# pythonmailer/financial-rag-system

Hardware: AMD Instinct MI355X
Metric: queries/sec + recall@5, batch=32 over 10Mx384 corpus (higher is better)
Workload: dtype fp16

## Files before the change

### financial-rag-system_amd/csrc/certify_kernels.hip

```cpp
namespace ragmi {

constexpr int kCandCap = 256;
constexpr int kBandLists = 32;
constexpr int kBandLists6 = 128;

template <typename IdT>
__device__ __forceinline__ void merge4_top32(const float (&ws)[4][32], const IdT (&wi)[4][32],
                                             int lane, IdT none, float& s, IdT& id) {
  s = lane < 32 ? ws[0][lane] : kNegInf;
  id = lane < 32 ? wi[0][lane] : none;
  for (int v = 1; v < 4; ++v) {
    if (lane >= 32) {
      s = ws[v][63 - lane];
      id = wi[v][63 - lane];
    }
    bitonic_merge64(s, id, lane);
  }
}

template <int D, int NC>
__device__ __forceinline__ void exact_scores_pairs(const half8* __restrict__ corpus,
                                                   const int (&rows)[NC],
                                                   const int (&qoff)[NC],
                                                   const float* __restrict__ qn, int lane,
                                                   float (&out)[NC],
                                                   const float* __restrict__ rows32) {
  constexpr int S = steps<D>();
  double acc[NC];
#pragma unroll
  for (int i = 0; i < NC; ++i) acc[i] = 0.0;
  for (int c = lane; c < D / 8; c += 64) {
    float h[NC][8];
#pragma unroll
    for (int i = 0; i < NC; ++i) {
      const int row = rows[i] < 0 ? 0 : rows[i];
      if (rows32) {
        const float4* p = reinterpret_cast<const float4*>(rows32 + (int64_t)row * D + 8 * c);
        const float4 u = p[0], v = p[1];
        h[i][0] = u.x; h[i][1] = u.y; h[i][2] = u.z; h[i][3] = u.w;
        h[i][4] = v.x; h[i][5] = v.y; h[i][6] = v.z; h[i][7] = v.w;
      } else {
        const half8 x =
            corpus[(int64_t)(row >> 4) * (S * 64) + (c >> 2) * 64 + (c & 3) * 16 + (row & 15)];
#pragma unroll
        for (int j = 0; j < 8; ++j) h[i][j] = (float)x[j];
      }
    }
#pragma unroll
    for (int i = 0; i < NC; ++i) {
      const float* qq = qn + qoff[i];
      const float4 qa = *reinterpret_cast<const float4*>(qq + 8 * c);
      const float4 qb = *reinterpret_cast<const float4*>(qq + 8 * c + 4);
      double x = acc[i];
      x = fma((double)h[i][0], (double)qa.x, x);
      x = fma((double)h[i][1], (double)qa.y, x);
      x = fma((double)h[i][2], (double)qa.z, x);
      x = fma((double)h[i][3], (double)qa.w, x);
      x = fma((double)h[i][4], (double)qb.x, x);
      x = fma((double)h[i][5], (double)qb.y, x);
      x = fma((double)h[i][6], (double)qb.z, x);
      x = fma((double)h[i][7], (double)qb.w, x);
      acc[i] = x;
    }
  }
#pragma unroll
  for (int d = 32; d > 0; d >>= 1) {
#pragma unroll
    for (int i = 0; i < NC; ++i) acc[i] = acc[i] + __shfl_xor(acc[i], d, 64);
  }
#pragma unroll
  for (int i = 0; i < NC; ++i)
    out[i] = rows[i] < 0 ? kNegInf : (float)__shfl(acc[i], 0, 64);
}

template <int D, int NC>
__device__ __forceinline__ void exact_scores_wave(const half8* __restrict__ corpus,
                                                  const int (&rows)[NC],
                                                  const float* __restrict__ qq, int lane,
                                                  float (&out)[NC],
                                                  const float* __restrict__ rows32) {
  int qoff[NC];
#pragma unroll
  for (int i = 0; i < NC; ++i) qoff[i] = 0;
  exact_scores_pairs<D, NC>(corpus, rows, qoff, qq, lane, out, rows32);
}

struct ExactStats {
  int* tier;
  unsigned long long* cnt;
  float* t2;
};

template <int D, bool FILTER, int BL = kBandLists>
__global__ __launch_bounds__(256) void select_kernel(const float* __restrict__ part_s,
                                                     const int* __restrict__ part_i,
                                                     const float* __restrict__ heads_s,
                                                     const int* __restrict__ heads_i,
                                                     const int* __restrict__ heads_n,
                                                     int n_lists,
                                                     const half8* __restrict__ corpus,
                                                     const uint32_t* __restrict__ tags,
                                                     const uint32_t* __restrict__ filt,
                                                     const half8* __restrict__ qfrag,
                                                     int n_rows,
                                                     const float* __restrict__ qn, int k,
                                                     const float* __restrict__ eps,
                                                     const float* __restrict__ seed_thr,
                                                     ExactStats fb, int64_t id_offset,
                                                     float* __restrict__ out_s,
                                                     int64_t* __restrict__ out_i,
                                                     int32_t* __restrict__ out_packed,
                                                     const float* __restrict__ rows32,
                                                     const float* __restrict__ eps_t2 = nullptr) {
  __shared__ float w_s[4][32];
  __shared__ int64_t w_i[4][32];
  __shared__ int sel[32];
  __shared__ int sel_n[32];
  __shared__ float cand_s[kCandCap];
  __shared__ int64_t cand_i[kCandCap];
  __shared__ int n_cand;
  __shared__ float head_t;
  __shared__ float c_s[4][32];
  __shared__ int c_i[4][32];
  __shared__ float e_s[32];
  __shared__ int e_i[32];
  __shared__ int qlist[kMaxLists];
  __shared__ int n_q;
  __shared__ int band[BL * kKS];
  __shared__ int n_band;
  __shared__ float n_s[2][32];
  __shared__ int n_i[2][32];
  __shared__ int verdict;
  __shared__ float floor_L, floor_E;
  const int bq = blockIdx.x, grp = bq / kQ, b = bq % kQ;
  const int tid = threadIdx.x, lane = tid & 63, wid = tid >> 6;
  const float eps_q = eps[bq], seed_q = seed_thr[bq];
  part_s += (int64_t)grp * n_lists * (kQ * kKS);
  part_i += (int64_t)grp * n_lists * (kQ * kKS);
  heads_s += (int64_t)grp * kQ * n_lists;
  heads_i += (int64_t)grp * kQ * n_lists;
  heads_n += (int64_t)grp * kQ * n_lists;
  auto at = [&](int l, int pos) { return ((int64_t)l * kQ + b) * kKS + pos; };

  constexpr int kCols = kMaxLists / 256;
  static_assert(kMaxLists <= 2048, "list index packs into 11 bits");
  auto hid = [](int row, int l) { return ((int64_t)row << 11) | (int64_t)l; };
  constexpr int64_t kId64None = INT64_MAX;
  float hs[kCols];
  int64_t hr[kCols];
#pragma unroll
  for (int j = 0; j < kCols; ++j) {
    const int l = min((j * 4 + wid) * 64 + lane, n_lists - 1);
    hs[j] = heads_s[(int64_t)b * n_lists + l];
    hr[j] = hid(heads_i[(int64_t)b * n_lists + l], l);
  }
  float lmax = kNegInf;
#pragma unroll
  for (int j = 0; j < kCols; ++j) {
    const int l = (j * 4 + wid) * 64 + lane;
    const bool ok = l < n_lists && hs[j] != kNegInf;
    hs[j] = ok ? hs[j] : kNegInf;
    hr[j] = ok ? hr[j] : kId64None;
    lmax = fmaxf(lmax, hs[j]);
  }
  {
    float m = lmax;
    int id = tid;
    bitonic_sort64(m, id, lane);
    if (lane < 32) w_s[wid][lane] = m;
  }
  if (tid == 0) {
    n_cand = 0;
    n_q = 0;
    n_band = 0;
    verdict = 0;
  }
  __syncthreads();
  if (wid == 0) {
    float m = lane < 32 ? w_s[0][lane] : kNegInf;
    int id = lane;
    for (int v = 1; v < 4; ++v) {
      if (lane >= 32) {
        m = w_s[v][63 - lane];
        id = 64 * v + lane;
      }
      bitonic_merge64(m, id, lane);
    }
    const float t32 = __shfl(m, 31, 64);
    if (lane == 0) head_t = t32;
  }
  __syncthreads();
  {
    const float T = head_t;
#pragma unroll
    for (int j = 0; j < kCols; ++j) {
      if (hs[j] != kNegInf && hs[j] >= T) {
        const int p = atomicAdd(&n_cand, 1);
        if (p < kCandCap) {
          cand_s[p] = hs[j];
          cand_i[p] = hr[j];
        }
      }
    }
  }
  __syncthreads();
  const int nc = n_cand;
  if (nc <= kCandCap) {
    float m = kNegInf;
    int64_t id = kId64None;
    if (64 * wid + lane < nc) {
      m = cand_s[64 * wid + lane];
// ... 31 lines not shown
      w_i[wid][lane] = ci;
    }
  }
  __syncthreads();
  if (wid == 0) {
    float x;
    int64_t id;
    merge4_top32(w_s, w_i, lane, kId64None, x, id);
    if (lane < 32) {
      const int l = (x != kNegInf) ? (int)(id & 2047) : -1;
      sel[lane] = l;
      sel_n[lane] = l >= 0 ? heads_n[(int64_t)b * n_lists + l] : 0;
    }
  }
  __syncthreads();

  {
    float ls[8];
    int li[8];
#pragma unroll
    for (int j = 0; j < 8; ++j) {
      const int l = sel[wid * 8 + j];
      const int pos = (j == 0 ? lane : 63 - lane) & (kKS - 1);
      const int64_t off = at(l < 0 ? 0 : l, pos);
      ls[j] = part_s[off];
      li[j] = part_i[off];
    }
#pragma unroll
    for (int j = 0; j < 8; ++j) {
      const int pos = (j == 0 ? lane : 63 - lane) & (kKS - 1);
      const bool use = sel[wid * 8 + j] >= 0 && ((j == 0) ? lane < 32 : lane >= 32) &&
                       pos < sel_n[wid * 8 + j];
      ls[j] = use ? ls[j] : kNegInf;
      li[j] = use ? li[j] : kIdNone32;
    }
    float s = ls[0];
    int id = li[0];
#pragma unroll
    for (int j = 1; j < 8; ++j) {
      if (lane >= 32) {
        s = ls[j];
        id = li[j];
      }
      bitonic_merge64(s, id, lane);
    }
    if (lane < 32) {
      c_s[wid][lane] = s;
      c_i[wid][lane] = id;
    }
  }
  __syncthreads();
  if (wid == 0) {
    float s;
    int id;
    merge4_top32(c_s, c_i, lane, kIdNone32, s, id);
    if (lane < 32) {
      c_s[0][lane] = s;
      c_i[0][lane] = id;
    }
  }
  __syncthreads();

  const float* qq = qn + (int64_t)bq * D;
  {
    int rows[8];
    float es[8];
#pragma unroll
    for (int j = 0; j < 8; ++j) {
      const int c = wid * 8 + j;
      rows[j] = c_s[0][c] != kNegInf ? c_i[0][c] : -1;
    }
    exact_scores_wave<D, 8>(corpus, rows, qq, lane, es, rows32);
    if (lane == 0) {
#pragma unroll
      for (int j = 0; j < 8; ++j) {
        e_s[wid * 8 + j] = es[j];
        e_i[wid * 8 + j] = rows[j] >= 0 ? rows[j] : kIdNone32;
      }
    }
  }
  __syncthreads();

  auto emit = [&](float s, int id) {
    if (lane < k) {
      const bool ok = s != kNegInf;
      if (out_packed) {
        out_packed[((int64_t)bq * k + lane) * 2] = __float_as_int(s);
        out_packed[((int64_t)bq * k + lane) * 2 + 1] = ok ? (int32_t)(id + id_offset) : -1;
      } else {
        out_s[(int64_t)bq * k + lane] = s;
        out_i[(int64_t)bq * k + lane] = ok ? (int64_t)id + id_offset : (int64_t)-1;
      }
    }
  };

  float rs = kNegInf;
  int ri = kIdNone32;
  if (wid == 0) {
    if (lane < 32) {
      rs = e_s[lane];
      ri = e_i[lane];
    }
    bitonic_sort64(rs, ri, lane);
    int v = 0;
    {
      const float ek = __shfl(rs, k - 1, 64);
      const float a32 = c_s[0][kKS - 1];
      float L = 0.0f;
      if (!(a32 == kNegInf || ek > a32 + eps_q)) {
        L = ek - eps_q;
        v = (L >= seed_q) ? 1 : 2;
      }
      if (lane == 0) {
        verdict = v;
        floor_L = L;
        floor_E = ek;
      }
    }
    if (v == 0) {
      emit(rs, ri);
      if (lane == 0) fb.tier[bq] = 0;
    }
  }
  __syncthreads();
  if (verdict == 0) return;

  const float L = floor_L;
  const bool seeded = verdict == 1;
  if (seeded) {
#pragma unroll
    for (int j = 0; j < kCols; ++j)
      if (hs[j] != kNegInf && hs[j] >= L) qlist[atomicAdd(&n_q, 1)] = (j * 4 + wid) * 64 + lane;
  }
  __syncthreads();
  const int nql = seeded ? n_q : 0;
  const int a_row = e_i[lane & 31];
  int rnd = 0;
  for (int c0 = 0; c0 < nql; c0 += BL) {
    constexpr int kG = BL / 8;
    const int pos = lane & (kKS - 1);
    float gs[kG];
    int gi[kG], gn[kG];
#pragma unroll
    for (int j = 0; j < kG; ++j) {
      const int l = qlist[min(c0 + (2 * j + (lane >> 5)) * 4 + wid, nql - 1)];
      gs[j] = part_s[at(l, pos)];
      gi[j] = part_i[at(l, pos)];
      gn[j] = heads_n[(int64_t)b * n_lists + l];
    }
#pragma unroll
    for (int j = 0; j < kG; ++j) {
      const bool in = c0 + (2 * j + (lane >> 5)) * 4 + wid < nql && pos < gn[j] && gs[j] >= L;
      if (in && gn[j] >= kKS && pos == kKS - 1) verdict = 2;
      bool in_a = false;
#pragma unroll
      for (int t = 0; t < 32; ++t) in_a |= gi[j] == __builtin_amdgcn_readlane(a_row, t);
      if (in && !in_a) band[atomicAdd(&n_band, 1)] = gi[j];
    }
    __syncthreads();
    if (verdict == 2) break;
    const int nb = n_band;
    for (int r0 = 0; r0 < nb; r0 += 32, ++rnd) {
      int rows[8];
      float es[8];
#pragma unroll
      for (int j = 0; j < 8; ++j) {
        const int c = r0 + wid * 8 + j;
        const int r = band[min(c, nb - 1)];
        rows[j] = c < nb ? r : -1;
      }
      exact_scores_wave<D, 8>(corpus, rows, qq, lane, es, rows32);
      if (lane == 0) {
#pragma unroll
        for (int j = 0; j < 8; ++j) {
          n_s[rnd & 1][wid * 8 + j] = es[j];
          n_i[rnd & 1][wid * 8 + j] = rows[j] >= 0 ? rows[j] : kIdNone32;
        }
      }
      __syncthreads();
      if (wid == 0) {
        if (lane >= 32) {
          rs = n_s[rnd & 1][lane - 32];
          ri = n_i[rnd & 1][lane - 32];
        }
        bitonic_sort64(rs, ri, lane);
      }
    }
    if (c0 + BL < nql) {
      __syncthreads();
      if (tid == 0) n_band = 0;
      __syncthreads();
    }
  }
  if (verdict == 2) {
    if (tid == 0) {
      fb.tier[bq] = 2;
      fb.t2[2 * bq] = eps_t2 ? floor_E - eps_t2[bq] : L;
      fb.t2[2 * bq + 1] = floor_E;
      atomicAdd(&fb.cnt[1], 1ull);
    }
    return;
  }
  if (tid == 0) {
    fb.tier[bq] = 1;
    atomicAdd(&fb.cnt[0], 1ull);
  }
  if (wid == 0) emit(rs, ri);
}

constexpr int kRescanMaxWG = 512;
constexpr int kRescanQ = 16;

__device__ __forceinline__ float exact_tree(double (&p)[16]) {
#pragma unroll
  for (int d = 8; d > 0; d >>= 1) {
#pragma unroll
    for (int i = 0; i < d; ++i) p[i] = p[i] + p[i + d];
  }
  double y = p[0] + __shfl_xor(p[0], 32, 64);
  y = y + __shfl_xor(y, 16, 64);
  return (float)y;
}

template <int D, bool F32>
__device__ __forceinline__ float exact_tile_scores(const half8* __restrict__ corpus,
                                                   const float* __restrict__ rows32, int t,
                                                   const float* __restrict__ qq, int lane) {
  constexpr int S = steps<D>();
  const int h = lane >> 4, r = lane & 15;
  double p[16];
#pragma unroll
  for (int i = 0; i < 16; ++i) p[i] = 0.0;
  int zoff = 0;
  asm volatile("" : "+v"(zoff));
  const half8* tp = corpus + (int64_t)t * (S * 64) + lane;
  const float* rp = F32 ? rows32 + ((int64_t)t * kTileRows + r) * D + 8 * h : nullptr;
  const float* qp = qq + 8 * h;
  constexpr int G = 2;
#pragma unroll
  for (int s0 = 0; s0 < S; s0 += G) {
    float x[G][8];
    float4 qa[G], qb[G];
#pragma unroll
    for (int g = 0; g < G; ++g) {
      const int s = s0 + g;
      if constexpr (F32) {
        const float4 u = *reinterpret_cast<const float4*>(rp + 32 * s + zoff);
        const float4 v = *reinterpret_cast<const float4*>(rp + 32 * s + 4 + zoff);
        x[g][0] = u.x; x[g][1] = u.y; x[g][2] = u.z; x[g][3] = u.w;
        x[g][4] = v.x; x[g][5] = v.y; x[g][6] = v.z; x[g][7] = v.w;
      } else {
        const half8 v = tp[s * 64 + zoff];
#pragma unroll
        for (int i = 0; i < 8; ++i) x[g][i] = (float)v[i];
      }
      qa[g] = *reinterpret_cast<const float4*>(qp + 32 * s + zoff);
      qb[g] = *reinterpret_cast<const float4*>(qp + 32 * s + 4 + zoff);
    }
#pragma unroll
    for (int g = 0; g < G; ++g) {
      double a = p[(s0 + g) & 15];
      a = fma((double)x[g][0], (double)qa[g].x, a);
      a = fma((double)x[g][1], (double)qa[g].y, a);
      a = fma((double)x[g][2], (double)qa[g].z, a);
      a = fma((double)x[g][3], (double)qa[g].w, a);
      a = fma((double)x[g][4], (double)qb[g].x, a);
      a = fma((double)x[g][5], (double)qb[g].y, a);
      a = fma((double)x[g][6], (double)qb[g].z, a);
      a = fma((double)x[g][7], (double)qb[g].w, a);
      p[(s0 + g) & 15] = a;
    }
    asm volatile("" : "+v"(zoff) : "v"(p[(s0 + G - 1) & 15]));
  }
  return exact_tree(p);
}

template <int D>
__device__ __forceinline__ float exact_tile_scores_reg(const half8 (&a)[steps<D>()],
                                                       const double* qd, int lane) {
  constexpr int S = steps<D>();
  static_assert(S <= 16, "one chunk per canonical lane");
  const int h = lane >> 4;
  double p[16];
#pragma unroll
  for (int i = 0; i < 16; ++i) p[i] = 0.0;
  int zoff = 0;
  asm volatile("" : "+v"(zoff));
  constexpr int G = 2;
#pragma unroll
  for (int s0 = 0; s0 < S; s0 += G) {
// ... 315 lines not shown
```

### financial-rag-system_amd/csrc/index_host.hpp

```cpp
#pragma once

#include <algorithm>
#include <array>
#include <cmath>
#include <mutex>
#include <type_traits>
#include <vector>

#include "common_host.hpp"
#include "device_common.hpp"

namespace ragmi {

constexpr int kRing = 8;
constexpr int kMaxGroups = 4;

struct Workspace {
  float* qn = nullptr;
  half8* qfrag = nullptr;
  uint32_t* filt = nullptr;
  float* smax = nullptr;
  float* seed = nullptr;
  float* part_s = nullptr;
  int* part_i = nullptr;
  float* heads_s = nullptr;
  int* heads_i = nullptr;
  int* heads_n = nullptr;
  int* progress = nullptr;
  float* eps = nullptr;
  int* fb_tier = nullptr;
  unsigned long long* fb_cnt = nullptr;
  int* tileq = nullptr;
  float* t2 = nullptr;
  float* t2_s = nullptr;
  int* t2_i = nullptr;
  int* t2_tk = nullptr;
  char* qfrag8 = nullptr;
  float* qp8 = nullptr;
  float* eps8 = nullptr;
  float* lk_smax = nullptr;
  float* lk_thr = nullptr;
  int* lk_cnt = nullptr;
  int* lk_again = nullptr;
  int* lk_need = nullptr;
  int* lk_cand = nullptr;
  float* lk_es = nullptr;
  hipEvent_t ev_in = nullptr;
  hipEvent_t ev_out = nullptr;
  hipStream_t owner = nullptr;
  int cus = 0;
  uint64_t cus_gen = 0;
  bool used = false;
  uint64_t tick = 0;
};

struct ProfPair {
  hipEvent_t a, b;
};

struct ViewSlot {
  uint32_t* p = nullptr;
  size_t bytes = 0;
  hipStream_t owner = nullptr;
  bool used = false;
  uint64_t tick = 0;
};

struct PassArgs {
  const float* q;
  int Bq, k;
  const uint32_t* filt;
  const uint32_t* tags;
  int64_t id_offset;
  float* out_s;
  int64_t* out_i;
  int32_t* out_packed;
};

template <typename F>
auto with_flag(bool on, F&& f) {
  if (on) return f(std::bool_constant<true>{});
  return f(std::bool_constant<false>{});
}
template <typename F>
auto with_filter(const uint32_t* filt, F&& f) {
  return with_flag(filt != nullptr, static_cast<F&&>(f));
}

template <typename F>
int with_dim(int dim, F&& f) {
  if (dim == 384) return f(std::integral_constant<int, 384>{});
  if (dim == 1024) return f(std::integral_constant<int, 1024>{});
  return fail(RAG_EINVAL, "unsupported dim (built: 384, 1024)");
}

enum CopyKind : int { kNoCopy = -1, kCopy8 = 0, kCopy6 = 1 };
constexpr int kCopies = 2;
struct ScanCopy {
  char* data = nullptr;
  float* meta = nullptr;
};

struct Copy8;
struct Copy6;
template <typename T>
struct type_tag {
  using type = T;
};
template <typename F>
auto with_copy(CopyKind kind, F&& f) {
  if (kind == kCopy6) return f(type_tag<Copy6>{});
  return f(type_tag<Copy8>{});
}

template <typename Slot, size_t N>
Slot* pick_slot(Slot (&slots)[N], hipStream_t st, Slot*& lru) {
  lru = &slots[0];
  for (auto& s : slots)
    if (s.tick < lru->tick) lru = &s;
  for (auto& s : slots)
    if (s.used && s.owner == st) return &s;
  for (auto& s : slots)
// ... 106 lines not shown
```

### financial-rag-system_amd/csrc/index_search.hip

```cpp
#include "index_host.hpp"
#include "prep_kernels.hip"
#include "scan_kernels.hip"
#include "seed_kernels.hip"
#include "certify_kernels.hip"
#include "merge_kernels.hip"
#include "largek_kernels.hip"
#include "reselect_kernels.hip"
#include "formula_kernels.hip"

#include <hipcub/hipcub.hpp>

using namespace ragmi;

namespace {

template <typename F>
int time_launches(int reps, F&& one, double* avg_ms) {
  EventPair ev;
  RAG_HIP(ev.create());
  one();
  RAG_HIP(hipEventRecord(ev.a, nullptr));
  for (int r = 0; r < reps; ++r) one();
  RAG_HIP(hipEventRecord(ev.b, nullptr));
  RAG_HIP(hipEventSynchronize(ev.b));
  float ms = 0.f;
  RAG_HIP(hipEventElapsedTime(&ms, ev.a, ev.b));
  RAG_HIP(hipGetLastError());
  *avg_ms = ms / reps;
  return RAG_OK;
}

hipError_t sort_pairs_desc(void* tmp, size_t tmp_bytes, const uint32_t* k_in, uint32_t* k_out,
                           const int* v_in, int* v_out, int n, hipStream_t st) {
  return hipcub::DeviceRadixSort::SortPairsDescending(tmp, tmp_bytes, k_in, k_out, v_in, v_out, n,
                                                      0, 32, st);
}

std::array<WsBuf, 7> lk_buffers(Workspace& w) {
  const size_t Q = kQ;
  return {ws_buf(w.lk_smax, Q * kLkSampleMax * 4), ws_buf(w.lk_thr, Q * 4),
          ws_buf(w.lk_cnt, Q * 4),                 ws_buf(w.lk_again, Q * 4),
          ws_buf(w.lk_need, 64),                   ws_buf(w.lk_cand, Q * kLkCap * 4),
          ws_buf(w.lk_es, Q * kLkCap * 4)};
}

std::array<WsBuf, 22> ws_buffers(const rag_index* h, Workspace& w) {
  const size_t G = (size_t)h->groups, Q = kQ, dim = (size_t)h->dim;
  const size_t max_lists = (size_t)std::min(h->max_wgs * kWavesPerWG, kMaxLists);
  return {ws_buf(w.qn, G * Q * dim * 4),
          ws_buf(w.qfrag, G * 2 * (dim / 32) * 64 * 16),
          ws_buf(w.filt, G * Q * 2 * 4),
          ws_buf(w.smax, G * (dim > 384 ? kMaxSampleWide : kMaxSample) * Q * 4),
          ws_buf(w.heads_s, G * kMaxLists * Q * 4),
          ws_buf(w.heads_i, G * kMaxLists * Q * 4),
          ws_buf(w.heads_n, G * kMaxLists * Q * 4),
          ws_buf(w.seed, G * Q * 4),
          ws_buf(w.part_s, G * max_lists * Q * kKS * 4),
          ws_buf(w.part_i, G * max_lists * Q * kKS * 4),
          ws_buf(w.progress, G * kMaxLists * 4),
          ws_buf(w.eps, G * Q * 4),
          ws_buf(w.fb_tier, G * Q * 4, true),
          ws_buf(w.fb_cnt, 32, true),
          ws_buf(w.tileq, 8 * kTileQStride * 4, true),
          ws_buf(w.t2, G * Q * 2 * 4),
          ws_buf(w.t2_s, G * Q * kRescanMaxWG * 32 * 4),
          ws_buf(w.t2_i, G * Q * kRescanMaxWG * 32 * 4),
          ws_buf(w.t2_tk, 64, true),
          ws_buf(w.qfrag8, h->copy[kCopy8].data ? 4 * (dim / 64) * 64 * 16 : 0),
          ws_buf(w.qp8, h->copy[kCopy8].data ? Q * 4 * 4 : 0),
          ws_buf(w.eps8, h->copy[kCopy8].data ? Q * 4 : 0)};
}

double store_eps(const rag_index* h) {
  if (h->storage != RAG_STORE_FP32) return 0.0;
  return (0x1p-11 * (1.0 + 0x1p-20) + 0x1p-25 * std::sqrt((double)h->dim)) * (1.0 + 0x1p-20);
}

std::atomic<uint64_t> g_stream_gen{1};

int stream_cus(const rag_index* h, hipStream_t st) {
  if (!st) return h->n_cu;
  uint32_t mask[32] = {};
  const uint32_t words = (uint32_t)std::min(32, (h->n_cu + 31) / 32);
  if (hipExtStreamGetCUMask(st, words, mask) != hipSuccess) {
    (void)hipGetLastError();
    return h->n_cu;
  }
  int n = 0;
  for (uint32_t i = 0; i < words; ++i) n += __builtin_popcount(mask[i]);
  return n > 0 && n < h->n_cu ? n : h->n_cu;
}

bool fused_prep() {
  static ragmi::Knob k("RAGMI_FUSED_PREP");
  return k.get(1) != 0;
}

int rescan_grid(const rag_index* h) {
  static ragmi::Knob k("RAGMI_RESCAN_WG");
  const int cap = k.get(kRescanMaxWG);
  if (cap <= 0) return 0;
  const int64_t n_tiles = (h->count + 15) / 16;
  return (int)std::max<int64_t>(1, std::min<int64_t>({(int64_t)cap, (int64_t)kRescanMaxWG,
                                                      (int64_t)h->n_cu, n_tiles / 128}));
}

int sample_div() {
  static ragmi::Knob k("RAGMI_SAMPLE_DIV");
  return std::max(1, k.get(128));
}

int seed_sample(int n_tiles, int cap) {
  return std::min({n_tiles, std::max(256, n_tiles / sample_div()), cap});
}

template <int D, bool FILTER>
void launch_seed(rag_index* h, Workspace& w, int groups, const uint32_t* tags, hipStream_t st) {
  const int n_tiles = (int)((h->count + 15) / 16);
  if (n_tiles == 0) return;
  constexpr int kCap = D > 384 ? kMaxSampleWide : kMaxSample;
  const int n_sample = seed_sample(n_tiles, kCap);
  if constexpr (D > 384)
    sample_wide_kernel<D, FILTER><<<dim3((n_sample + 7) / 8), dim3(256), 0, st>>>(
        h->corpus, tags, w.filt, w.qfrag, (int)h->count, n_tiles, n_sample, w.smax, groups);
  else
    sample_kernel<D, FILTER><<<dim3((n_sample + 7) / 8, groups), dim3(256), 0, st>>>(
        h->corpus, tags, w.filt, w.qfrag, (int)h->count, n_tiles, n_sample, w.smax);
  thresh_kernel<kCap><<<dim3(kQ, groups), dim3(256), 0, st>>>(w.smax, n_sample, w.eps, w.seed);
}

template <int D, bool FILTER>
void launch_prep_seed(rag_index* h, Workspace& w, const float* q, int Bq, const uint32_t* filt_in,
                      const uint32_t* tags, hipStream_t st) {
  if constexpr (D <= 384) {
    const int n_tiles = (int)((h->count + 15) / 16);
    const int n_sample = seed_sample(n_tiles, kMaxSample);
    qprep_sample_kernel<D, FILTER><<<dim3(std::max(1, (n_sample + 7) / 8)), dim3(256), 0, st>>>(
        q, Bq, filt_in, w.qn, w.qfrag, w.filt, w.eps, store_eps(h), h->corpus, tags,
        (int)h->count, n_tiles, n_sample, w.smax);
    if (n_sample > 0)
      thresh_kernel<kMaxSample><<<dim3(kQ, 1), dim3(256), 0, st>>>(w.smax, n_sample, w.eps,
                                                                  w.seed);
  }
}

bool use_prescan(const rag_index* h, int k) {
  return h->copy[kCopy8].data && RAG_PRESCAN_ROUTES(h->prescan, h->dim, h->storage, k, h->count);
}

bool use_prescan6(const rag_index* h, int k) {
  return h->copy[kCopy6].data && RAG_PRESCAN6_ROUTES(h->prescan, h->dim, h->storage, k, h->count);
}

CopyKind pass_copy(const rag_index* h, int k) {
  if (!use_prescan(h, k)) return kNoCopy;
  return use_prescan6(h, k) ? kCopy6 : kCopy8;
}

template <int D>
void launch_prep8(rag_index* h, Workspace& w, const float* q, int Bq, const uint32_t* filt,
                  const uint32_t* tags, hipStream_t st, CopyKind kind) {
  qprep8_kernel<D><<<dim3(kQ), dim3(64), 0, st>>>(q, Bq, filt, w.qn, w.qfrag, w.filt, w.eps,
                                                  w.qfrag8, w.qp8, w.eps8);
  const int nt = (int)((h->count + 15) / 16);
  if (nt == 0) return;
  const int n_sample = seed_sample(nt, kMaxSample);
  with_filter(filt, [&](auto f) {
    with_copy(kind, [&](auto c) {
      sample_kernel_q<D, decltype(f)::value, typename decltype(c)::type>
          <<<dim3((n_sample + 7) / 8), dim3(256), 0, st>>>(
              h->copy[kind].data, h->copy[kind].meta, tags, w.filt,
              reinterpret_cast<const intx4*>(w.qfrag8), w.qp8, (int)h->count, nt, n_sample,
              w.smax);
    });
  });
  thresh_kernel<kMaxSample><<<dim3(kQ, 1), dim3(256), 0, st>>>(w.smax, n_sample, w.eps8, w.seed);
}

bool partitioned(const rag_index* h, int cus) { return cus > 0 && cus < h->n_cu; }
int max_wgs_on(const rag_index* h, int cus) { return partitioned(h, cus) ? 2 * cus : h->max_wgs; }

int scan_grid(const rag_index* h, int cus, bool filtered, CopyKind copy) {
  static ragmi::Knob k_wgs("RAGMI_SCAN_WGS");
  const int wg_env = k_wgs.get(0) > 0 ? std::max(8, k_wgs.get(0)) : 0;
  const bool part = partitioned(h, cus);
  const int max_wgs = max_wgs_on(h, cus);
  const int wg_cap = wg_env ? wg_env
                     : (filtered && copy == kNoCopy) ? max_wgs
// ... 55 lines not shown
    if (h->scan_any && h->scan_last != st) RAG_HIP(hipStreamWaitEvent(st, h->scan_done, 0));
  } else if (h->serial_scans == 2) {
    if (!h->scan_stream) RAG_HIP(hipStreamCreateWithFlags(&h->scan_stream, hipStreamNonBlocking));
    if (!w.ev_in) RAG_HIP(hipEventCreateWithFlags(&w.ev_in, hipEventDisableTiming));
    if (!w.ev_out) RAG_HIP(hipEventCreateWithFlags(&w.ev_out, hipEventDisableTiming));
    RAG_HIP(hipEventRecord(w.ev_in, st));
    RAG_HIP(hipStreamWaitEvent(h->scan_stream, w.ev_in, 0));
    st = h->scan_stream;
  }
  ProfPair pp{};
  const bool timed = h->prof > 0 && (h->prof_seq++ % h->prof) == 0;
  if (timed) {
    RAG_HIP(hipEventCreate(&pp.a));
    RAG_HIP(hipEventCreate(&pp.b));
    if constexpr (kLdsQ) RAG_HIP(hipEventRecord(pp.a, st));
  }
  const auto with_scan_args = [&](auto&& go, auto... tail) {
    return go(h->corpus, a.tags, w.filt, w.qfrag, (int)h->count, (int)n_tiles, w.seed, w.part_s,
              w.part_i, w.heads_s, w.heads_i, w.heads_n, tail...);
  };
  const bool wide = kLdsQ && groups > 1 && !filt;
  if (wide) {
    static ragmi::Knob k_wide("RAGMI_WIDE_WGS");
    const int wide_env = k_wide.get(0) > 0 ? std::max(8, k_wide.get(0)) : 0;
    const int cap = wide_env ? std::min(wide_env, max_wgs / 2) : max_wgs / 2;
    grid = (int)std::min<int64_t>(cap, std::max<int64_t>(1, n_tiles));
  }
  if constexpr (kLdsQ) {
    const dim3 g3(grid * groups);
    if (wide) {
      launch_fixed<kWideBlock>(scan_wide_kernel<D, 0, true>, dim3(grid), 0, st, h->corpus,
                               w.qfrag, (int)h->count, (int)n_tiles, w.seed, w.part_s,
                               w.part_i, w.heads_s, w.heads_i, w.heads_n, groups);
    } else {
      if (groups > 1)
        RAG_HIP(hipMemsetAsync(w.progress, 0, (size_t)grid * kLdsWaves * groups * 4, st));
      const auto launch = [&](auto nt) {
        with_filter(filt, [&](auto f) {
          with_scan_args(
              [&](auto... args) {
                launch_fixed<kLdsBlock>(
                    scan_lds_kernel<D, decltype(f)::value, decltype(nt)::value>, g3, 0, st,
                    args...);
              },
              groups, w.progress);
        });
      };
      if (groups == 1)
        launch(std::true_type{});
      else
        launch(std::false_type{});
    }
  } else {
    const int rc = with_filter(filt, [&](auto f) -> int {
      constexpr bool F = decltype(f)::value;
      if constexpr (D == 384) {
        const auto with_copy_args = [&](auto&& go) {
          return go(h->copy[copy].data, h->copy[copy].meta, a.tags, w.filt,
                    reinterpret_cast<const intx4*>(w.qfrag8), w.qp8, (int)h->count, (int)n_tiles,
                    w.seed, w.part_s, w.part_i, w.heads_s, w.heads_i, w.heads_n);
        };
        if (copy == kCopy6) return with_copy_args(RAG_SCAN_GO(scan_kernel_i6<D, F>));
        if (copy == kCopy8) return with_copy_args(RAG_SCAN_GO(scan_kernel_i8<D, F>));
      }
      return with_scan_args(RAG_SCAN_GO(scan_kernel<D, F>), nullptr);
    });
    if (rc) return rc;
  }
  if (timed) {
    if constexpr (kLdsQ) RAG_HIP(hipEventRecord(pp.b, st));
    h->prof_pairs.push_back(pp);
  }
  if (h->serial_scans == 1) {
    RAG_HIP(hipEventRecord(h->scan_done, st));
    h->scan_last = st;
    h->scan_any = true;
  } else if (h->serial_scans == 2) {
    RAG_HIP(hipEventRecord(w.ev_out, st));
    RAG_HIP(hipStreamWaitEvent(caller, w.ev_out, 0));
    st = caller;
  }
  const int n_lists = wide ? grid : grid * (kLdsQ ? kLdsWaves : kWavesPerWG);
  const ExactStats fb{w.fb_tier, w.fb_cnt, w.t2};
  with_filter(filt, [&](auto f) {
    with_flag(copy == kCopy6, [&](auto six) {
      constexpr int BL = (D == 384 && decltype(six)::value) ? kBandLists6 : kBandLists;
      select_kernel<D, decltype(f)::value, BL><<<dim3(Bq), dim3(256), 0, st>>>(
          w.part_s, w.part_i, w.heads_s, w.heads_i, w.heads_n, n_lists, h->corpus, a.tags, w.filt,
          w.qfrag, (int)h->count, w.qn, a.k, copy != kNoCopy ? w.eps8 : w.eps, w.seed, fb,
          a.id_offset, a.out_s, a.out_i, a.out_packed, h->rows32,
          copy != kNoCopy ? w.eps : nullptr);
    });
  });
  const int R = std::min(rescan_grid(h), part ? w.cus : h->n_cu);
  if (R > 0) {
    with_filter(filt, [&](auto f) {
      launch_fixed<kScanBlock>(rescan_kernel<D, decltype(f)::value>, dim3(R), 0, st, w.fb_tier,
                               w.t2, Bq, h->corpus, a.tags, w.filt, w.qfrag, (int)h->count, w.qn,
                               a.k, w.eps, w.t2_s, w.t2_i, w.t2_tk, a.id_offset, a.out_s, a.out_i,
                               a.out_packed, h->rows32);
    });
  } else {
    mark_unanswered_kernel<<<dim3(1), dim3(64), 0, st>>>(w.fb_tier, Bq, w.fb_cnt);
  }
  RAG_HIP(hipGetLastError());
  return RAG_OK;
}
#undef RAG_SCAN_GO

int ensure_lk(Workspace& w) {
  if (w.lk_cand) return RAG_OK;
  if (ragmi::ws_alloc_all(lk_buffers(w)) != hipSuccess) {
    (void)hipGetLastError();
    return ragmi::fail(RAG_ENOMEM, "large-k workspace allocation failed");
  }
  return RAG_OK;
}

template <int D>
int launch_full_pass(rag_index* h, Workspace& w, const PassArgs& a, hipStream_t st) {
  const int Bq = a.Bq, k = a.k;
  qprep_kernel<D><<<dim3(kQ), dim3(64), 0, st>>>(a.q, Bq, a.filt, w.qn, w.qfrag, w.filt, w.eps,
                                                  store_eps(h));
  RAG_HIP(hipGetLastError());
  const int n = (int)h->count;
  auto emit = [&](int j, const uint32_t* keys, const int* rows, const int* n_match) {
    full_emit_kernel<<<dim3((unsigned)std::min<int64_t>(1024, (k + 255) / 256)), dim3(256), 0,
                       st>>>(keys, rows, n_match, k, a.id_offset,
                             a.out_s ? a.out_s + (int64_t)j * k : nullptr,
                             a.out_i ? a.out_i + (int64_t)j * k : nullptr,
                             a.out_packed ? a.out_packed + (int64_t)j * k * 2 : nullptr);
  };
  StreamScratch scratch(st);
  if (n == 0) {
    RAG_HIP(scratch.alloc(4));
    int* zero = reinterpret_cast<int*>(scratch.p);
    RAG_HIP(hipMemsetAsync(zero, 0, 4, st));
    for (int j = 0; j < Bq; ++j) emit(j, nullptr, nullptr, zero);
    RAG_HIP(hipGetLastError());
    return RAG_OK;
  }
  size_t tmp_bytes = 0;
  RAG_HIP(hipcub::DeviceRadixSort::SortPairsDescending(
      nullptr, tmp_bytes, static_cast<const uint32_t*>(nullptr), static_cast<uint32_t*>(nullptr),
      static_cast<const int*>(nullptr), static_cast<int*>(nullptr), n, 0, 32, st));
  const size_t nb = (size_t)n * 4;
  const size_t m_off = 4 * nb, t_off = m_off + 256;
  RAG_HIP(scratch.alloc(t_off + tmp_bytes));
  char* const buf = scratch.p;
  uint32_t* k_in = reinterpret_cast<uint32_t*>(buf);
  uint32_t* k_out = reinterpret_cast<uint32_t*>(buf + nb);
  int* v_in = reinterpret_cast<int*>(buf + 2 * nb);
  int* v_out = reinterpret_cast<int*>(buf + 3 * nb);
  int* n_match = reinterpret_cast<int*>(buf + m_off);
  void* tmp = buf + t_off;
  RAG_HIP(hipMemsetAsync(n_match, 0, 4 * kQ, st));
  const int grid = (int)std::max<int64_t>(1, std::min<int64_t>(8 * h->n_cu, (n + 31) / 32));
  int rc = RAG_OK;
  for (int j = 0; j < Bq && rc == RAG_OK; ++j) {
    with_filter(a.filt, [&](auto f) {
      constexpr bool F = decltype(f)::value;
      full_score_kernel<D, F><<<dim3(grid), dim3(256), 0, st>>>(
          h->corpus, a.tags, F ? w.filt + 2 * j : nullptr, w.qn + (int64_t)j * D, n, h->rows32,
          k_in, v_in, n_match + j);
    });
    if (hipGetLastError() != hipSuccess ||
        sort_pairs_desc(tmp, tmp_bytes, k_in, k_out, v_in, v_out, n, st) != hipSuccess) {
      rc = ragmi::fail(RAG_EHIP, "full exact pass: score / sort launch failed");
      break;
    }
    emit(j, k_out, v_out, n_match + j);
    if (hipGetLastError() != hipSuccess) rc = ragmi::fail(RAG_EHIP, "full exact pass: emit");
  }
  (void)hipMemsetAsync(w.fb_tier, 0, 4 * kQ, st);
  return rc;
}
// ... 859 lines not shown
```

Measured before the change: 63220.

## Split band rescoring of select kernel into a multi-slice band kernel

For the D=384 six-bit copy path, the select kernel now stops after seeding. It writes its candidate list, floor and current top-32 to a per-query workspace record. A new band_kernel then spreads each query's band rescoring across several workgroups (slices), and the last slice merges the published partial top-32 lists using an atomic ticket. This replaces one block per query walking the whole band serially, raising parallelism with batch=32, at the cost of an extra launch, global workspace traffic and fence-based cross-block sync.

New measurement: 68240 (median of 6 runs). 7.9% higher.

```diff
diff --git a/financial-rag-system_amd/csrc/certify_kernels.hip b/financial-rag-system_amd/csrc/certify_kernels.hip
--- a/financial-rag-system_amd/csrc/certify_kernels.hip
+++ b/financial-rag-system_amd/csrc/certify_kernels.hip
@@ -3,6 +3,16 @@
 constexpr int kCandCap = 256;
 constexpr int kBandLists = 32;
 constexpr int kBandLists6 = 128;
+constexpr int kBandHead = 0;
+constexpr int kBandSlicesMax = 16;
+constexpr int kBandRecHdr = 96;
+constexpr int kBandRec = kBandRecHdr + kMaxLists;
+constexpr int kBandPub = 72;
+struct BandWs {
+  int* rec;
+  int* pub;
+  int* tk;
+};
 
 template <typename IdT>
 __device__ __forceinline__ void merge4_top32(const float (&ws)[4][32], const IdT (&wi)[4][32],
@@ -90,6 +100,100 @@
   unsigned long long* cnt;
   float* t2;
 };
+
+__device__ __forceinline__ void emit_topk(float s, int id, int lane, int bq, int k,
+                                          int64_t id_offset, float* __restrict__ out_s,
+                                          int64_t* __restrict__ out_i,
+                                          int32_t* __restrict__ out_packed) {
+  if (lane < k) {
+    const bool ok = s != kNegInf;
+    if (out_packed) {
+      out_packed[((int64_t)bq * k + lane) * 2] = __float_as_int(s);
+      out_packed[((int64_t)bq * k + lane) * 2 + 1] = ok ? (int32_t)(id + id_offset) : -1;
+    } else {
+      out_s[(int64_t)bq * k + lane] = s;
+      out_i[(int64_t)bq * k + lane] = ok ? (int64_t)id + id_offset : (int64_t)-1;
+    }
+  }
+}
+
+__device__ __forceinline__ void hand_to_tier2(const ExactStats& fb, int bq, float L, float e_k,
+                                              const float* __restrict__ eps_t2) {
+  fb.tier[bq] = 2;
+  fb.t2[2 * bq] = eps_t2 ? e_k - eps_t2[bq] : L;
+  fb.t2[2 * bq + 1] = e_k;
+  atomicAdd(&fb.cnt[1], 1ull);
+}
+
+template <int D, int BL, typename ListP>
+__device__ __forceinline__ bool band_chunk(ListP qlist, int c0, int nql, bool more,
+                                           const float* __restrict__ part_s,
+                                           const int* __restrict__ part_i,
+                                           const int* __restrict__ heads_n, int n_lists, int b,
+                                           float L, int a_row, const half8* __restrict__ corpus,
+                                           const float* __restrict__ qq,
+                                           const float* __restrict__ rows32,
+                                           int (&band)[BL * kKS], int& n_band,
+                                           float (&n_s)[2][32], int (&n_i)[2][32], int& verdict,
+                                           float& rs, int& ri, int& rnd) {
+  const int tid = threadIdx.x, lane = tid & 63, wid = tid >> 6;
+  auto at = [&](int l, int pos) { return ((int64_t)l * kQ + b) * kKS + pos; };
+  constexpr int kG = BL / 8;
+  const int pos = lane & (kKS - 1);
+  float gs[kG];
+  int gi[kG], gn[kG];
+#pragma unroll
+  for (int j = 0; j < kG; ++j) {
+    const int l = qlist[min(c0 + (2 * j + (lane >> 5)) * 4 + wid, nql - 1)];
+    gs[j] = part_s[at(l, pos)];
+    gi[j] = part_i[at(l, pos)];
+    gn[j] = heads_n[(int64_t)b * n_lists + l];
+  }
+#pragma unroll
+  for (int j = 0; j < kG; ++j) {
+    const bool in = c0 + (2 * j + (lane >> 5)) * 4 + wid < nql && pos < gn[j] && gs[j] >= L;
+    if (in && gn[j] >= kKS && pos == kKS - 1) verdict = 2;
+    bool in_a = false;
+#pragma unroll
+    for (int t = 0; t < 32; ++t) in_a |= gi[j] == __builtin_amdgcn_readlane(a_row, t);
+    if (in && !in_a) band[atomicAdd(&n_band, 1)] = gi[j];
+  }
+  __syncthreads();
+  if (verdict == 2) return false;
+  const int nb = n_band;
+  for (int r0 = 0; r0 < nb; r0 += 32, ++rnd) {
+    int rows[8];
+    float es[8];
+#pragma unroll
+    for (int j = 0; j < 8; ++j) {
+      const int c = r0 + wid * 8 + j;
+      const int r = band[min(c, nb - 1)];
+      rows[j] = c < nb ? r : -1;
+    }
+    exact_scores_wave<D, 8>(corpus, rows, qq, lane, es, rows32);
+    if (lane == 0) {
+#pragma unroll
+      for (int j = 0; j < 8; ++j) {
+        n_s[rnd & 1][wid * 8 + j] = es[j];
+        n_i[rnd & 1][wid * 8 + j] = rows[j] >= 0 ? rows[j] : kIdNone32;
+      }
+    }
+    __syncthreads();
+    if (wid == 0) {
+      if (lane >= 32) {
+        rs = n_s[rnd & 1][lane - 32];
+        ri = n_i[rnd & 1][lane - 32];
+      }
+      bitonic_sort64(rs, ri, lane);
+    }
+  }
+  if (more) {
+    __syncthreads();
+    if (tid == 0) n_band = 0;
+    __syncthreads();
+  }
+  return true;
+}
 
 template <int D, bool FILTER, int BL = kBandLists>
 __global__ __launch_bounds__(256) void select_kernel(const float* __restrict__ part_s,
@@ -111,7 +215,10 @@
                                                      int64_t* __restrict__ out_i,
                                                      int32_t* __restrict__ out_packed,
                                                      const float* __restrict__ rows32,
-                                                     const float* __restrict__ eps_t2 = nullptr) {
+                                                     const float* __restrict__ eps_t2 = nullptr,
+                                                     BandWs bw = {}) {
+  constexpr bool kHead = BL == kBandHead;
+  constexpr int kChunk = kHead ? kBandLists : BL;
   __shared__ float w_s[4][32];
   __shared__ int64_t w_i[4][32];
   __shared__ int sel[32];
@@ -126,7 +233,7 @@
   __shared__ int e_i[32];
   __shared__ int qlist[kMaxLists];
   __shared__ int n_q;
-  __shared__ int band[BL * kKS];
+  __shared__ int band[kChunk * kKS];
   __shared__ int n_band;
   __shared__ float n_s[2][32];
   __shared__ int n_i[2][32];
@@ -324,16 +431,7 @@
   __syncthreads();
 
   auto emit = [&](float s, int id) {
-    if (lane < k) {
-      const bool ok = s != kNegInf;
-      if (out_packed) {
-        out_packed[((int64_t)bq * k + lane) * 2] = __float_as_int(s);
-        out_packed[((int64_t)bq * k + lane) * 2 + 1] = ok ? (int32_t)(id + id_offset) : -1;
-      } else {
-        out_s[(int64_t)bq * k + lane] = s;
-        out_i[(int64_t)bq * k + lane] = ok ? (int64_t)id + id_offset : (int64_t)-1;
-      }
-    }
+    emit_topk(s, id, lane, bq, k, id_offset, out_s, out_i, out_packed);
   };
 
   float rs = kNegInf;
@@ -363,9 +461,37 @@
       emit(rs, ri);
       if (lane == 0) fb.tier[bq] = 0;
     }
+    if constexpr (kHead) {
+      int* rq = bw.rec + (int64_t)bq * kBandRec;
+      if (lane < 32 && v == 1) {
+        rq[32 + lane] = __float_as_int(rs);
+        rq[64 + lane] = ri;
+      }
+      if (lane == 0 && v != 1) rq[0] = -1;
+    }
   }
   __syncthreads();
   if (verdict == 0) return;
+  if constexpr (kHead) {
+    int* rq = bw.rec + (int64_t)bq * kBandRec;
+    if (verdict == 1) {
+#pragma unroll
+      for (int j = 0; j < kCols; ++j)
+        if (hs[j] != kNegInf && hs[j] >= floor_L)
+          rq[kBandRecHdr + atomicAdd(&n_q, 1)] = (j * 4 + wid) * 64 + lane;
+      __syncthreads();
+    }
+    if (tid == 0) {
+      if (verdict == 1) {
+        rq[0] = n_q;
+        rq[1] = __float_as_int(floor_L);
+        rq[2] = __float_as_int(floor_E);
+      } else {
+        hand_to_tier2(fb, bq, floor_L, floor_E, eps_t2);
+      }
+    }
+    return;
+  }
 
   const float L = floor_L;
   const bool seeded = verdict == 1;
@@ -378,69 +504,13 @@
   const int nql = seeded ? n_q : 0;
   const int a_row = e_i[lane & 31];
   int rnd = 0;
-  for (int c0 = 0; c0 < nql; c0 += BL) {
-    constexpr int kG = BL / 8;
-    const int pos = lane & (kKS - 1);
-    float gs[kG];
-    int gi[kG], gn[kG];
-#pragma unroll
-    for (int j = 0; j < kG; ++j) {
-      const int l = qlist[min(c0 + (2 * j + (lane >> 5)) * 4 + wid, nql - 1)];
-      gs[j] = part_s[at(l, pos)];
-      gi[j] = part_i[at(l, pos)];
-      gn[j] = heads_n[(int64_t)b * n_lists + l];
-    }
-#pragma unroll
-    for (int j = 0; j < kG; ++j) {
-      const bool in = c0 + (2 * j + (lane >> 5)) * 4 + wid < nql && pos < gn[j] && gs[j] >= L;
-      if (in && gn[j] >= kKS && pos == kKS - 1) verdict = 2;
-      bool in_a = false;
-#pragma unroll
-      for (int t = 0; t < 32; ++t) in_a |= gi[j] == __builtin_amdgcn_readlane(a_row, t);
-      if (in && !in_a) band[atomicAdd(&n_band, 1)] = gi[j];
-    }
-    __syncthreads();
-    if (verdict == 2) break;
-    const int nb = n_band;
-    for (int r0 = 0; r0 < nb; r0 += 32, ++rnd) {
-      int rows[8];
-      float es[8];
-#pragma unroll
-      for (int j = 0; j < 8; ++j) {
-        const int c = r0 + wid * 8 + j;
-        const int r = band[min(c, nb - 1)];
-        rows[j] = c < nb ? r : -1;
-      }
-      exact_scores_wave<D, 8>(corpus, rows, qq, lane, es, rows32);
-      if (lane == 0) {
-#pragma unroll
-        for (int j = 0; j < 8; ++j) {
-          n_s[rnd & 1][wid * 8 + j] = es[j];
-          n_i[rnd & 1][wid * 8 + j] = rows[j] >= 0 ? rows[j] : kIdNone32;
-        }
-      }
-      __syncthreads();
-      if (wid == 0) {
-        if (lane >= 32) {
-          rs = n_s[rnd & 1][lane - 32];
-          ri = n_i[rnd & 1][lane - 32];
-        }
-        bitonic_sort64(rs, ri, lane);
-      }
-    }
-    if (c0 + BL < nql) {
-      __syncthreads();
-      if (tid == 0) n_band = 0;
-      __syncthreads();
-    }
-  }
+  for (int c0 = 0; c0 < nql; c0 += kChunk)
+    if (!band_chunk<D, kChunk>(qlist, c0, nql, c0 + kChunk < nql, part_s, part_i, heads_n, n_lists,
+                               b, L, a_row, corpus, qq, rows32, band, n_band, n_s, n_i, verdict,
+                               rs, ri, rnd))
+      break;
   if (verdict == 2) {
-    if (tid == 0) {
-      fb.tier[bq] = 2;
-      fb.t2[2 * bq] = eps_t2 ? floor_E - eps_t2[bq] : L;
-      fb.t2[2 * bq + 1] = floor_E;
-      atomicAdd(&fb.cnt[1], 1ull);
-    }
+    if (tid == 0) hand_to_tier2(fb, bq, L, floor_E, eps_t2);
     return;
   }
   if (tid == 0) {
@@ -448,6 +518,108 @@
     atomicAdd(&fb.cnt[0], 1ull);
   }
   if (wid == 0) emit(rs, ri);
+}
+
+template <int D>
+__global__ __launch_bounds__(256) void band_kernel(const float* __restrict__ part_s,
+                                                   const int* __restrict__ part_i,
+                                                   const int* __restrict__ heads_n, int n_lists,
+                                                   const half8* __restrict__ corpus,
+                                                   const float* __restrict__ qn, int k,
+                                                   BandWs bw, ExactStats fb,
+                                                   const float* __restrict__ eps_t2,
+                                                   int64_t id_offset, float* __restrict__ out_s,
+                                                   int64_t* __restrict__ out_i,
+                                                   int32_t* __restrict__ out_packed,
+                                                   const float* __restrict__ rows32) {
+  __shared__ int band[kBandLists * kKS];
+  __shared__ int n_band;
+  __shared__ float n_s[2][32];
+  __shared__ int n_i[2][32];
+  __shared__ int verdict;
+  __shared__ int last;
+  const int S = gridDim.x, s = blockIdx.x, bq = blockIdx.y, grp = bq / kQ, b = bq % kQ;
+  const int tid = threadIdx.x, lane = tid & 63, wid = tid >> 6;
+  const int* rq = bw.rec + (int64_t)bq * kBandRec;
+  const int nql = rq[0];
+  if (nql < 0) return;
+  const float L = __int_as_float(rq[1]), floor_E = __int_as_float(rq[2]);
+  const int a_row = rq[64 + (lane & 31)];
+  part_s += (int64_t)grp * n_lists * (kQ * kKS);
+  part_i += (int64_t)grp * n_lists * (kQ * kKS);
+  heads_n += (int64_t)grp * kQ * n_lists;
+  const float* qq = qn + (int64_t)bq * D;
+  if (tid == 0) {
+    n_band = 0;
+    verdict = 1;
+  }
+  __syncthreads();
+  float rs = kNegInf;
+  int ri = kIdNone32;
+  int rnd = 0;
+  constexpr int BL = kBandLists;
+  for (int c0 = s * BL; c0 < nql; c0 += S * BL)
+    if (!band_chunk<D, BL>(rq + kBandRecHdr, c0, nql, c0 + S * BL < nql, part_s, part_i, heads_n,
+                           n_lists, b, L, a_row, corpus, qq, rows32, band, n_band, n_s, n_i,
+                           verdict, rs, ri, rnd))
+      break;
+  int* pub = bw.pub + ((int64_t)bq * kBandSlicesMax + s) * kBandPub;
+  if (wid == 0 && lane < 32) {
+    pub[lane] = __float_as_int(rs);
+    pub[32 + lane] = ri;
+  }
+  if (tid == 0) pub[64] = verdict == 2;
+  asm volatile("s_waitcnt vmcnt(0)" ::: "memory");
+  __syncthreads();
+  if (tid == 0) {
+    __builtin_amdgcn_fence(__ATOMIC_RELEASE, "agent");
+    asm volatile("s_waitcnt vmcnt(0)" ::: "memory");
+    last = atomicAdd(&bw.tk[bq], 1) == S - 1;
+  }
+  __syncthreads();
+  if (!last) return;
+  if (tid == 0) {
+    __builtin_amdgcn_fence(__ATOMIC_ACQUIRE, "agent");
+    asm volatile("s_waitcnt vmcnt(0)" ::: "memory");
+  }
+  __syncthreads();
+  if (wid != 0) return;
+  const int* pq = bw.pub + (int64_t)bq * kBandSlicesMax * kBandPub;
+  const bool full = __ballot(lane < S && pq[(lane < S ? lane : 0) * kBandPub + 64] != 0) != 0;
+  if (full) {
+    if (lane == 0) hand_to_tier2(fb, bq, L, floor_E, eps_t2);
+  } else {
+    float x = lane < 32 ? __int_as_float(rq[32 + lane]) : kNegInf;
+    int id = lane < 32 ? rq[64 + lane] : kIdNone32;
+    constexpr int kPf = 8;
+    for (int u0 = 0; u0 < S; u0 += kPf) {
+      float xs[kPf];
+      int is[kPf];
+#pragma unroll
+      for (int u = 0; u < kPf; ++u) {
+        const int* p = pq + min(u0 + u, S - 1) * kBandPub + (lane >= 32 ? 63 - lane : 0);
+        const bool use = u0 + u < S && lane >= 32;
+        xs[u] = use ? __int_as_float(p[0]) : kNegInf;
+        is[u] = use ? p[32] : kIdNone32;
+      }
+#pragma unroll
+      for (int u = 0; u < kPf; ++u) {
+        const float head = __shfl(xs[u], 63, 64), t32 = __shfl(x, 31, 64);
+        if (head < t32 || head == kNegInf) continue;
+        if (lane >= 32) {
+          x = xs[u];
+          id = is[u];
+        }
+        bitonic_merge64(x, id, lane);
+      }
+    }
+    emit_topk(x, id, lane, bq, k, id_offset, out_s, out_i, out_packed);
+    if (lane == 0) {
+      fb.tier[bq] = 1;
+      atomicAdd(&fb.cnt[0], 1ull);
+    }
+  }
+  if (lane == 0) bw.tk[bq] = 0;
 }
 
 constexpr int kRescanMaxWG = 512;
diff --git a/financial-rag-system_amd/csrc/index_host.hpp b/financial-rag-system_amd/csrc/index_host.hpp
--- a/financial-rag-system_amd/csrc/index_host.hpp
+++ b/financial-rag-system_amd/csrc/index_host.hpp
@@ -38,6 +38,9 @@
   char* qfrag8 = nullptr;
   float* qp8 = nullptr;
   float* eps8 = nullptr;
+  int* bd_rec = nullptr;
+  int* bd_pub = nullptr;
+  int* bd_tk = nullptr;
   float* lk_smax = nullptr;
   float* lk_thr = nullptr;
   int* lk_cnt = nullptr;
diff --git a/financial-rag-system_amd/csrc/index_search.hip b/financial-rag-system_amd/csrc/index_search.hip
--- a/financial-rag-system_amd/csrc/index_search.hip
+++ b/financial-rag-system_amd/csrc/index_search.hip
@@ -44,7 +44,7 @@
           ws_buf(w.lk_es, Q * kLkCap * 4)};
 }
 
-std::array<WsBuf, 22> ws_buffers(const rag_index* h, Workspace& w) {
+std::array<WsBuf, 25> ws_buffers(const rag_index* h, Workspace& w) {
   const size_t G = (size_t)h->groups, Q = kQ, dim = (size_t)h->dim;
   const size_t max_lists = (size_t)std::min(h->max_wgs * kWavesPerWG, kMaxLists);
   return {ws_buf(w.qn, G * Q * dim * 4),
@@ -68,7 +68,10 @@
           ws_buf(w.t2_tk, 64, true),
           ws_buf(w.qfrag8, h->copy[kCopy8].data ? 4 * (dim / 64) * 64 * 16 : 0),
           ws_buf(w.qp8, h->copy[kCopy8].data ? Q * 4 * 4 : 0),
-          ws_buf(w.eps8, h->copy[kCopy8].data ? Q * 4 : 0)};
+          ws_buf(w.eps8, h->copy[kCopy8].data ? Q * 4 : 0),
+          ws_buf(w.bd_rec, h->copy[kCopy8].data ? Q * kBandRec * 4 : 0),
+          ws_buf(w.bd_pub, h->copy[kCopy8].data ? Q * kBandSlicesMax * kBandPub * 4 : 0),
+          ws_buf(w.bd_tk, h->copy[kCopy8].data ? Q * 4 : 0, true)};
 }
 
 double store_eps(const rag_index* h) {
@@ -104,6 +107,9 @@
   return (int)std::max<int64_t>(1, std::min<int64_t>({(int64_t)cap, (int64_t)kRescanMaxWG,
                                                       (int64_t)h->n_cu, n_tiles / 128}));
 }
+
+constexpr int kBandSlices = 4;
+static_assert(kBandSlices >= 0 && kBandSlices <= kBandSlicesMax, "bd_pub holds kBandSlicesMax lists");
 
 int sample_div() {
   static ragmi::Knob k("RAGMI_SAMPLE_DIV");
@@ -325,16 +331,25 @@
   }
   const int n_lists = wide ? grid : grid * (kLdsQ ? kLdsWaves : kWavesPerWG);
   const ExactStats fb{w.fb_tier, w.fb_cnt, w.t2};
+  const BandWs bw{w.bd_rec, w.bd_pub, w.bd_tk};
   with_filter(filt, [&](auto f) {
     with_flag(copy == kCopy6, [&](auto six) {
-      constexpr int BL = (D == 384 && decltype(six)::value) ? kBandLists6 : kBandLists;
+      constexpr int BL = !(D == 384 && decltype(six)::value) ? kBandLists
+                         : kBandSlices > 0                   ? kBandHead
+                                                             : kBandLists6;
       select_kernel<D, decltype(f)::value, BL><<<dim3(Bq), dim3(256), 0, st>>>(
           w.part_s, w.part_i, w.heads_s, w.heads_i, w.heads_n, n_lists, h->corpus, a.tags, w.filt,
           w.qfrag, (int)h->count, w.qn, a.k, copy != kNoCopy ? w.eps8 : w.eps, w.seed, fb,
           a.id_offset, a.out_s, a.out_i, a.out_packed, h->rows32,
-          copy != kNoCopy ? w.eps : nullptr);
+          copy != kNoCopy ? w.eps : nullptr, bw);
     });
   });
+  if constexpr (D == 384 && kBandSlices > 0) {
+    if (copy == kCopy6)
+      band_kernel<D><<<dim3(kBandSlices, Bq), dim3(256), 0, st>>>(
+          w.part_s, w.part_i, w.heads_n, n_lists, h->corpus, w.qn, a.k, bw, fb, w.eps,
+          a.id_offset, a.out_s, a.out_i, a.out_packed, h->rows32);
+  }
   const int R = std::min(rescan_grid(h), part ? w.cus : h->n_cu);
   if (R > 0) {
     with_filter(filt, [&](auto f) {
```
